# lacibeb/GA3C

Hardware: NVIDIA B200
Metric: TPS: A3C training frames/s, NetworkVP 84x84x4 (PPS: predictions/s, in 'pps') (higher is better)
Workload: dtype bf16

## Files before the change

### ga3c_b200/csrc/common.cuh

```cuda
#pragma once
#include <cuda_runtime.h>
#include <cuda_bf16.h>
#include <stdint.h>

namespace ga3c {

constexpr int IMG = 84, IMG_C = 4, STATE_DIM = IMG * IMG * IMG_C;
constexpr int C1_OUT = 16, H1 = 21, N1_POS = H1 * H1;
constexpr int C2_OUT = 32, H2 = 11, N2_POS = H2 * H2;
constexpr int FLAT = N2_POS * C2_OUT;
constexpr int FC = 256;
constexpr int MAX_ACTIONS = 18;

constexpr int XS_W = 88, XS_ROW_BYTES = XS_W * 8, XS_BYTES = XS_W * XS_ROW_BYTES;
constexpr int N1P_W = 24, N1P_BYTES = N1P_W * N1P_W * 32;

constexpr int XB_QROWS = 128, XB_QUARTERS = 4, XB_PLANE_BYTES = XB_QROWS * 16, XB_QBYTES = 8 * XB_PLANE_BYTES,
              XB_FRAME_BYTES = XB_QUARTERS * XB_QBYTES, XB_LIVE_ROWS = 484;
constexpr int G_W = 13, G_ROWS = 172, G_LBO = G_ROWS * 16, G_BYTES = 4 * G_LBO;
constexpr int B2_ROWS = 160, B2_LBO = B2_ROWS * 16, B2_BYTES = 8 * B2_LBO;
__host__ __device__ constexpr int b2_pixel_offset(int y, int x, int h) {
  return ((((y + 1) & 1) * 2 + ((x + 1) & 1)) * 2 + h) * B2_LBO + (((y + 1) >> 1) * G_W + ((x + 1) >> 1)) * 16;
}
__host__ __device__ constexpr int g_pos_offset(int oy, int ox, int j) { return j * G_LBO + ((oy + 1) * G_W + ox + 1) * 16; }

__device__ __forceinline__ uint32_t smem_u32(const void* p) {
  return static_cast<uint32_t>(__cvta_generic_to_shared(p));
}

__device__ __forceinline__ uint32_t pack_bf16(float lo, float hi) {
  __nv_bfloat162 v = __floats2bfloat162_rn(lo, hi);
  return *reinterpret_cast<uint32_t*>(&v);
}
__device__ __forceinline__ float bf16_lo(uint32_t v) { return __uint_as_float(v << 16); }
__device__ __forceinline__ float bf16_hi(uint32_t v) { return __uint_as_float(v & 0xFFFF0000u); }

__device__ __forceinline__ void mma_bf16_16816(float (&d)[4], const uint32_t (&a)[4], uint32_t b0, uint32_t b1) {
  asm volatile(
      "mma.sync.aligned.m16n8k16.row.col.f32.bf16.bf16.f32 {%0,%1,%2,%3}, {%4,%5,%6,%7}, {%8,%9}, {%0,%1,%2,%3};\n"
      : "+f"(d[0]), "+f"(d[1]), "+f"(d[2]), "+f"(d[3])
      : "r"(a[0]), "r"(a[1]), "r"(a[2]), "r"(a[3]), "r"(b0), "r"(b1));
}

__device__ __forceinline__ void ldsm_x4(uint32_t (&r)[4], uint32_t addr) {
  asm volatile("ldmatrix.sync.aligned.m8n8.x4.shared.b16 {%0,%1,%2,%3}, [%4];\n"
               : "=r"(r[0]), "=r"(r[1]), "=r"(r[2]), "=r"(r[3]) : "r"(addr));
}
__device__ __forceinline__ void ldsm_x4_t(uint32_t (&r)[4], uint32_t addr) {
  asm volatile("ldmatrix.sync.aligned.m8n8.x4.trans.shared.b16 {%0,%1,%2,%3}, [%4];\n"
               : "=r"(r[0]), "=r"(r[1]), "=r"(r[2]), "=r"(r[3]) : "r"(addr));
}
__device__ __forceinline__ void lds64(uint32_t& a, uint32_t& b, uint32_t addr) {
  asm volatile("ld.shared.v2.u32 {%0,%1}, [%2];\n" : "=r"(a), "=r"(b) : "r"(addr));
}
__device__ __forceinline__ void lds128(uint32_t (&r)[4], uint32_t addr) {
  asm volatile("ld.shared.v4.u32 {%0,%1,%2,%3}, [%4];\n"
               : "=r"(r[0]), "=r"(r[1]), "=r"(r[2]), "=r"(r[3]) : "r"(addr));
}
__device__ __forceinline__ void sts32(uint32_t addr, uint32_t v) {
  asm volatile("st.shared.u32 [%0], %1;\n" ::"r"(addr), "r"(v));
}
__device__ __forceinline__ void sts64(uint32_t addr, uint32_t a, uint32_t b) {
  asm volatile("st.shared.v2.u32 [%0], {%1,%2};\n" ::"r"(addr), "r"(a), "r"(b));
}
__device__ __forceinline__ void sts128(uint32_t addr, uint4 v) {
  asm volatile("st.shared.v4.u32 [%0], {%1,%2,%3,%4};\n" ::"r"(addr), "r"(v.x), "r"(v.y), "r"(v.z), "r"(v.w));
}

__device__ __forceinline__ void cp_async16(uint32_t dst, const void* src, int src_bytes) {
  asm volatile("cp.async.cg.shared.global [%0], [%1], 16, %2;\n" ::"r"(dst), "l"(src), "r"(src_bytes));
}
__device__ __forceinline__ void cp_async4(uint32_t dst, const void* src, int src_bytes) {
  asm volatile("cp.async.ca.shared.global [%0], [%1], 4, %2;\n" ::"r"(dst), "l"(src), "r"(src_bytes));
}
__device__ __forceinline__ void cp_async_commit() { asm volatile("cp.async.commit_group;\n" ::); }
template <int N>
__device__ __forceinline__ void cp_async_wait() { asm volatile("cp.async.wait_group %0;\n" ::"n"(N)); }

__device__ __forceinline__ float4 ldg_stream(const float4* p) {
  float4 r;
  asm volatile("ld.global.nc.L1::no_allocate.v4.f32 {%0,%1,%2,%3}, [%4];\n"
               : "=f"(r.x), "=f"(r.y), "=f"(r.z), "=f"(r.w) : "l"(p));
  return r;
}

__device__ __forceinline__ void mbar_init(uint32_t bar, uint32_t count) {
  asm volatile("mbarrier.init.shared::cta.b64 [%0], %1;\n" ::"r"(bar), "r"(count));
}
__device__ __forceinline__ void mbar_expect_tx(uint32_t bar, uint32_t bytes) {
  asm volatile("mbarrier.arrive.expect_tx.shared::cta.b64 _, [%0], %1;\n" ::"r"(bar), "r"(bytes) : "memory");
}
__device__ __forceinline__ void mbar_wait(uint32_t bar, uint32_t parity) {
  asm volatile(
      "{\n"
      ".reg .pred p;\n"
      "WAIT_%=:\n"
      "mbarrier.try_wait.parity.shared::cta.b64 p, [%0], %1;\n"
      "@p bra DONE_%=;\n"
      "bra WAIT_%=;\n"
      "DONE_%=:\n"
      "}\n" ::"r"(bar), "r"(parity) : "memory");
}
__device__ __forceinline__ void bulk_load(uint32_t dst, const void* src, uint32_t bytes, uint32_t bar) {
  asm volatile("cp.async.bulk.shared::cluster.global.mbarrier::complete_tx::bytes [%0], [%1], %2, [%3];\n" ::"r"(dst),
               "l"(src), "r"(bytes), "r"(bar)
               : "memory");
}
__device__ __forceinline__ uint64_t l2_policy_evict_first() {
  uint64_t p;
  asm volatile("createpolicy.fractional.L2::evict_first.b64 %0, 1.0;\n" : "=l"(p));
  return p;
}
__device__ __forceinline__ uint64_t l2_policy_evict_last() {
  uint64_t p;
  asm volatile("createpolicy.fractional.L2::evict_last.b64 %0, 1.0;\n" : "=l"(p));
  return p;
}
__device__ __forceinline__ uint64_t l2_policy_normal() {
  uint64_t p;
  asm volatile("createpolicy.fractional.L2::evict_normal.b64 %0, 1.0;\n" : "=l"(p));
  return p;
}
__device__ __forceinline__ void bulk_load_hint(uint32_t dst, const void* src, uint32_t bytes, uint32_t bar, uint64_t policy) {
  asm volatile("cp.async.bulk.shared::cluster.global.mbarrier::complete_tx::bytes.L2::cache_hint [%0], [%1], %2, [%3], %4;\n" ::"r"(dst),
               "l"(src), "r"(bytes), "r"(bar), "l"(policy)
               : "memory");
}
__device__ __forceinline__ void bulk_store_hint(void* dst, uint32_t src, uint32_t bytes, uint64_t policy) {
  asm volatile("cp.async.bulk.global.shared::cta.bulk_group.L2::cache_hint [%0], [%1], %2, %3;\n" ::"l"(dst), "r"(src), "r"(bytes),
               "l"(policy)
               : "memory");
}
__device__ __forceinline__ void stg128_hint(void* dst, uint4 v, uint64_t policy) {
  asm volatile("st.global.L2::cache_hint.v4.b32 [%0], {%1,%2,%3,%4}, %5;\n" ::"l"(dst), "r"(v.x), "r"(v.y), "r"(v.z), "r"(v.w), "l"(policy)
               : "memory");
}
__device__ __forceinline__ void bulk_store(void* dst, uint32_t src, uint32_t bytes) {
  asm volatile("cp.async.bulk.global.shared::cta.bulk_group [%0], [%1], %2;\n" ::"l"(dst), "r"(src), "r"(bytes) : "memory");
}
__device__ __forceinline__ void bulk_commit() { asm volatile("cp.async.bulk.commit_group;\n" ::: "memory"); }
__device__ __forceinline__ void bulk_wait_read0() { asm volatile("cp.async.bulk.wait_group.read 0;\n" ::: "memory"); }
__device__ __forceinline__ void fence_proxy_async() { asm volatile("fence.proxy.async.shared::cta;\n" ::: "memory"); }
__device__ __forceinline__ void fence_mbar_init() { asm volatile("fence.mbarrier_init.release.cluster;\n" ::: "memory"); }

constexpr int FRAME_BYTES = STATE_DIM * 4;
template <int NCH>
__device__ __forceinline__ void stg_issue_chunk(uint32_t stg, const float* frame, int c, uint32_t bars) {
  constexpr int CB = FRAME_BYTES / NCH, PARTS = 4 / NCH > 0 ? 4 / NCH : 1, PB = CB / PARTS;
  static_assert(CB * NCH == FRAME_BYTES && PB * PARTS == CB && PB % 16 == 0, "chunking must be exact and 16-B granular");
  mbar_expect_tx(bars + 8 * c, CB);
#pragma unroll
  for (int k = 0; k < PARTS; ++k)
    bulk_load(stg + c * CB + k * PB, reinterpret_cast<const uint8_t*>(frame) + c * CB + k * PB, PB, bars + 8 * c);
}

__device__ __forceinline__ void griddep_launch() { asm volatile("griddepcontrol.launch_dependents;\n" ::: "memory"); }

enum KernelId { K_CONV_FWD = 0, K_DENSE_FWD, K_HEADS, K_DENSE_WGRAD, K_DENSE_DGRAD, K_CONV12_BWD, K_CONV11_WGRAD, K_RMSPROP,
                K_GRAD_REDUCE, K_MLP_FUSED, K_MLP_WGRAD, K_MLP_REDUCE, K_DP_BIG, K_MLP_TC, K_HISTO,
                K_COUNT };
constexpr int TRACE_SLOTS = 6;
static __device__ unsigned long long* g_trace = nullptr;
__device__ __forceinline__ void trace_mark(int kid, int what) {
  if (threadIdx.x == 0) {
    unsigned long long* t = g_trace;
    if (t != nullptr) {
      unsigned long long now;
      asm volatile("mov.u64 %0, %%globaltimer;\n" : "=l"(now));
      atomicMin(t + kid * TRACE_SLOTS + 2 * what, now);
      atomicMax(t + kid * TRACE_SLOTS + 2 * what + 1, now);
    }
  }
}
__device__ __forceinline__ void trace_mark_by(int kid, int what, bool me) {
  if (me) {
    unsigned long long* t = g_trace;
    if (t != nullptr) {
      unsigned long long now;
      asm volatile("mov.u64 %0, %%globaltimer;\n" : "=l"(now));
      atomicMin(t + kid * TRACE_SLOTS + 2 * what, now);
      atomicMax(t + kid * TRACE_SLOTS + 2 * what + 1, now);
    }
  }
}
__device__ __forceinline__ void griddep_wait(int kid) {
  trace_mark(kid, 0);
  asm volatile("griddepcontrol.wait;\n" ::: "memory");
  trace_mark(kid, 1);
}
static __device__ unsigned long long* g_evt = nullptr;
constexpr unsigned int EVT_PER_WARP = 1024, EVT_WARPS = 16;
struct EvtLog {
  unsigned long long* base;
  unsigned int i;
};
__device__ __forceinline__ EvtLog evt_open() {
  EvtLog l;
  l.base = (blockIdx.x == 0 && (threadIdx.x & 31) == 0) ? g_evt : nullptr;
  l.i = 0;
  return l;
}
__device__ __forceinline__ void evt_mark(EvtLog& l, int id, int arg) {
  if (l.base != nullptr && l.i < EVT_PER_WARP) {
    unsigned long long now;
    asm volatile("mov.u64 %0, %%globaltimer;\n" : "=l"(now));
    const unsigned int slot = (threadIdx.x >> 5) * EVT_PER_WARP + l.i++;
    l.base[2 * slot] = now;
    l.base[2 * slot + 1] = ((unsigned long long)(threadIdx.x >> 5) << 32) | ((unsigned long long)id << 16) | (unsigned long long)(arg & 0xFFFF);
  }
}
#define GA3C_EVT_ATTACH(fn) \
  int fn(unsigned long long* buf) { return (int)cudaMemcpyToSymbol(g_evt, &buf, sizeof(buf)); }
#define GA3C_TRACE_ATTACH(fn)                                                                   \
  int fn(unsigned long long* buf) { return (int)cudaMemcpyToSymbol(g_trace, &buf, sizeof(buf)); }

template <class... KArgs, class... Args>
inline int launch_pdl(void (*kernel)(KArgs...), dim3 grid, dim3 block, size_t smem, cudaStream_t stream, Args... args) {
  cudaLaunchConfig_t cfg{};
  cfg.gridDim = grid; cfg.blockDim = block; cfg.dynamicSmemBytes = smem; cfg.stream = stream;
  cudaLaunchAttribute attr[1];
  attr[0].id = cudaLaunchAttributeProgrammaticStreamSerialization;
  attr[0].val.programmaticStreamSerializationAllowed = 1;
  cfg.attrs = attr; cfg.numAttrs = 1;
  return (int)cudaLaunchKernelEx(&cfg, kernel, static_cast<KArgs>(args)...);
}

__device__ __forceinline__ float warp_sum(float v) {
#pragma unroll
  for (int o = 16; o > 0; o >>= 1) v += __shfl_xor_sync(0xffffffffu, v, o);
  return v;
}

__device__ __forceinline__ int n1p_slot(int px) { return (px & ~7) | ((px >> 1) & 3) | ((px & 1) << 2); }
__device__ __forceinline__ int n1p_off(int py, int px, int chunk) {
  return ((py * N1P_W + n1p_slot(px)) << 5) + (((chunk ^ (px >> 3)) & 1) << 4);
}

template <int NT>
__device__ __forceinline__ void stage_frame_bf16(const float* __restrict__ x, uint32_t xs_base, int tid) {
  const float4* src = reinterpret_cast<const float4*>(x);
  constexpr int NPIX = IMG * IMG;
  constexpr int UNROLL = 7;
  for (int base = 0; base < NPIX; base += NT * UNROLL) {
    float4 v[UNROLL];
#pragma unroll
    for (int u = 0; u < UNROLL; ++u) {
      int i = base + u * NT + tid;
      if (i < NPIX) v[u] = ldg_stream(src + i);
    }
#pragma unroll
    for (int u = 0; u < UNROLL; ++u) {
      int i = base + u * NT + tid;
      if (i < NPIX) {
        int y = i / IMG, xx = i - y * IMG;
        sts64(xs_base + (y + 2) * XS_ROW_BYTES + (xx + 2) * 8, pack_bf16(v[u].x, v[u].y), pack_bf16(v[u].z, v[u].w));
      }
    }
  }
}

}
```

### ga3c_b200/csrc/conv_fwd.cu

```cuda
#include "common.cuh"
#include "kernels.h"
#include "tcgen05.cuh"
#include "conv_blk.cuh"

namespace ga3c {

constexpr int CF_THREADS = 512, CF_AUX_WARPS = 6, CF_ISSUE_WARP = 6, CF_STORE_WARP = 7, CF_EPI_WARP0 = 8;
static_assert(CF_EPI_WARP0 % 4 == 0, "epilogue warp e must own TMEM lane quarter e");
constexpr int C11_TILES = 4;
constexpr int C11_TSTRIDE = 127;
static_assert((C11_TILES - 1) * C11_TSTRIDE + 128 + BLK_W <= BLK_ROWS && C11_TILES * C11_TSTRIDE >= H1 * BLK_W, "tiles must cover the outputs and stay inside the buffer");

constexpr int CF_OFF_A2 = 0;
constexpr int CF_OFF_B2 = CF_OFF_A2 + 4 * 128 * 128;
constexpr int CF_OFF_BLK = CF_OFF_B2 + 4 * 32 * 128;
constexpr int CF_OFF_RING = CF_OFF_BLK + BLK_BYTES;
constexpr int CF_OFF_WQ = CF_OFF_RING + CF_AUX_WARPS * PW_SLOTS * PW_BYTES;
constexpr int CF_OFF_LUT = CF_OFF_WQ + 4 * 2048;
constexpr int CF_OFF_BIAS = CF_OFF_LUT + 3584;
constexpr int CF_OFF_BAR = CF_OFF_BIAS + (C1_OUT + C2_OUT) * 4;
constexpr int BAR_RING = 0;
constexpr int BAR_BLKRDY = 12;
constexpr int BAR_C11 = 16;
constexpr int BAR_T1FREE = 20;
constexpr int BAR_A2RDY = 24;
constexpr int BAR_MMA2 = 25;
constexpr int BAR_T2FREE = 26;
constexpr int BAR_STORED = 27;
constexpr int CF_NBAR = 31;
constexpr int CF_OFF_TSLOT = CF_OFF_BAR + CF_NBAR * 8;
constexpr int CF_OFF_XCH = CF_OFF_TSLOT + 16;
constexpr int CF_SMEM = CF_OFF_XCH + 1024 + 1024;
static_assert(CF_SMEM <= 232448, "shared memory budget of one CTA per SM");
constexpr int CF_TMEM_COLS = 256, TMEM_C12 = 128;

template <bool U8, bool EVT>
__global__ void __launch_bounds__(CF_THREADS, 1)
conv_fwd_kernel(const void* __restrict__ x, const float* __restrict__ w11, const float* __restrict__ b11,
                const float* __restrict__ w12, const float* __restrict__ b12,
                uint8_t* __restrict__ n1_out, uint8_t* __restrict__ xblk_out, uint16_t* __restrict__ n2_out, int batch, int hints) {
  extern __shared__ uint8_t smem_raw[];
  const uint32_t sbase = (smem_u32(smem_raw) + 1023u) & ~1023u;
  uint8_t* const smem = smem_raw + (sbase - smem_u32(smem_raw));
  const uint32_t sa2 = sbase + CF_OFF_A2, sb2 = sbase + CF_OFF_B2, blk = sbase + CF_OFF_BLK, ring = sbase + CF_OFF_RING,
                 wq = sbase + CF_OFF_WQ, lut = sbase + CF_OFF_LUT, bars = sbase + CF_OFF_BAR, tslot = sbase + CF_OFF_TSLOT;
  float* bias_s = reinterpret_cast<float*>(smem + CF_OFF_BIAS);
  const int tid = threadIdx.x, warp = tid >> 5, lane = tid & 31;
  EvtLog evt_i = EVT ? evt_open() : EvtLog{nullptr, 0};
  auto mark = [&](int id, int arg) { if (EVT) evt_mark(evt_i, id, arg); };
  const int stride = gridDim.x;
  const int n_frames = ((int)blockIdx.x < batch) ? (batch - 1 - (int)blockIdx.x) / stride + 1 : 0;
  const int n_chunks = n_frames * PW_NCHUNK;
  auto frame_of = [&](int k) { return (size_t)(blockIdx.x + k * stride); };
  auto bar = [&](int i) { return bars + i * 8; };
  const uint64_t pol_stream = (hints & 1) ? l2_policy_evict_first() : l2_policy_normal();
  const uint64_t pol_keep = (hints & 2) ? l2_policy_evict_last() : l2_policy_normal();
  auto issue_chunk = [&](int q, int slot) {
    const int k = q / PW_NCHUNK, c = q - k * PW_NCHUNK;
    constexpr uint32_t bytes = U8 ? PW_BYTES_U8 : PW_BYTES;
    mbar_expect_tx(bar(BAR_RING + slot), bytes);
    bulk_load_hint(ring + slot * PW_BYTES, static_cast<const uint8_t*>(x) + (frame_of(k) * PW_NCHUNK + c) * bytes, bytes,
                   bar(BAR_RING + slot), pol_stream);
  };

  mark(60, 0);
  if (tid == 0) {
    for (int i = 0; i < CF_AUX_WARPS * PW_SLOTS; ++i) mbar_init(bar(BAR_RING + i), 1);
    for (int i = 0; i < 4; ++i) {
      mbar_init(bar(BAR_BLKRDY + i), pw_group_chunks(i));
      mbar_init(bar(BAR_C11 + i), 1);
      mbar_init(bar(BAR_T1FREE + i), 4);
    }
    mbar_init(bar(BAR_A2RDY), 8);
    mbar_init(bar(BAR_MMA2), 1);
    mbar_init(bar(BAR_T2FREE), 4);
    for (int i = 0; i < 4; ++i) mbar_init(bar(BAR_STORED + i), 1);
    fence_mbar_init();
  }
  if (warp == CF_EPI_WARP0) tmem_alloc<CF_TMEM_COLS>(tslot);
  __syncthreads();
  mark(61, 0);
  if (warp < CF_AUX_WARPS && lane == 0)
    for (int j = 0; j < PW_SLOTS; ++j)
      if (warp + j * CF_AUX_WARPS < n_chunks) issue_chunk(warp + j * CF_AUX_WARPS, warp * PW_SLOTS + j);
  for (int i = tid; i < (CF_OFF_RING - CF_OFF_A2) / 16; i += CF_THREADS)
    if (i < CF_OFF_B2 / 16 || i >= CF_OFF_BLK / 16) sts128(sbase + i * 16, make_uint4(0, 0, 0, 0));
  for (int p = tid; p < N1_POS; p += CF_THREADS) {
    const int y = p / H1, xx = p - y * H1;
    uint32_t e[4];
#pragma unroll
    for (int idx = 0; idx < 4; ++idx) {
      const int kh = ((y + 1) & 1) + 2 * (idx >> 1), kw = ((xx + 1) & 1) + 2 * (idx & 1);
      const int oy2 = y + 1 - kh, ox2 = xx + 1 - kw;
      const bool ok = oy2 >= 0 && ox2 >= 0 && (oy2 >> 1) < H2 && (ox2 >> 1) < H2;
      const int row = kh * 128 + (oy2 >> 1) * H2 + (ox2 >> 1);
      e[idx] = ok ? (uint32_t)(row * 8 + ((2 * kw) ^ (row & 7))) : 0xFFFFu;
    }
    sts64(lut + p * 8, e[0] | (e[1] << 16), e[2] | (e[3] << 16));
  }
  fence_proxy_async();
  __syncthreads();
  mark(62, 0);
  griddep_launch();
  uint32_t tmem_base;
  asm volatile("ld.shared.u32 %0, [%1];\n" : "=r"(tmem_base) : "r"(tslot));
  if (warp >= CF_AUX_WARPS) {
    trace_mark_by(K_CONV_FWD, 0, tid == CF_AUX_WARPS * 32);
    asm volatile("griddepcontrol.wait;\n" ::: "memory");
    trace_mark_by(K_CONV_FWD, 1, tid == CF_AUX_WARPS * 32);
    mark(63, 0);
    const int t = tid - CF_AUX_WARPS * 32;
    float4 q12[8];
    float2 q11[8];
    const bool do12 = t < 256, do11 = t >= 64;
    const int kh = t >> 6, c12 = (t >> 3) & 7, n12 = (t & 7) * 4;
    if (do12) {
      const float* w = w12 + ((kh * 4 + (c12 >> 1)) * C1_OUT + (c12 & 1) * 8) * C2_OUT + n12;
#pragma unroll
      for (int e = 0; e < 8; ++e) q12[e] = *reinterpret_cast<const float4*>(w + e * C2_OUT);
    }
    const int i11 = t - 64, a11 = i11 >> 7, j11 = (i11 >> 4) & 7, b11i = (i11 >> 3) & 1, n11 = (i11 & 7) * 2;
    if (do11) {
      const float* w = w11 + (((4 * a11 + (j11 >> 1)) * 8 + 4 * b11i + (j11 & 1) * 2) * 4) * C1_OUT + n11;
#pragma unroll
      for (int e = 0; e < 8; ++e) q11[e] = *reinterpret_cast<const float2*>(w + e * C1_OUT);
    }
    if (t < C1_OUT) bias_s[t] = b11[t];
    if (t >= 32 && t < 32 + C2_OUT) bias_s[C1_OUT + t - 32] = b12[t - 32];
    if (do12) {
#pragma unroll
      for (int qn = 0; qn < 4; ++qn) {
        const int n = n12 + qn;
        auto f = [&](const float4& v) { return qn == 0 ? v.x : qn == 1 ? v.y : qn == 2 ? v.z : v.w; };
        sts128(sb2 + kh * 4096 + n * 128 + ((c12 ^ (n & 7)) << 4),
               make_uint4(pack_bf16(f(q12[0]), f(q12[1])), pack_bf16(f(q12[2]), f(q12[3])), pack_bf16(f(q12[4]), f(q12[5])),
                          pack_bf16(f(q12[6]), f(q12[7]))));
      }
    }
    if (do11) {
      const uint32_t dst = wq + a11 * 4096 + j11 * 512 + (b11i * 16 + n11) * 16;
      sts128(dst, make_uint4(pack_bf16(q11[0].x, q11[1].x), pack_bf16(q11[2].x, q11[3].x), pack_bf16(q11[4].x, q11[5].x),
                             pack_bf16(q11[6].x, q11[7].x)));
      sts128(dst + 16, make_uint4(pack_bf16(q11[0].y, q11[1].y), pack_bf16(q11[2].y, q11[3].y), pack_bf16(q11[4].y, q11[5].y),
                                  pack_bf16(q11[6].y, q11[7].y)));
    }
    fence_proxy_async();
    tc_fence_before();
    named_bar_sync(4, CF_THREADS - CF_AUX_WARPS * 32);
    tc_fence_after();
    mark(64, 0);
  }

  if (warp < CF_AUX_WARPS) {
    uint32_t lane_off[3];
    blk_lane_offsets(lane, lane_off);
    int j = 0;
#pragma unroll 1
    for (int q = warp; q < n_chunks; q += CF_AUX_WARPS, ++j) {
      const int k = q / PW_NCHUNK, c = q - k * PW_NCHUNK, slot = warp * PW_SLOTS + (j & 1);
      uint32_t pk[PW_ROWS][3][2];
      mbar_wait(bar(BAR_RING + slot), (j >> 1) & 1);
      blk_load_rows4<U8>(ring + slot * PW_BYTES, lane, pk);
      __syncwarp();
      if (lane == 0 && q + PW_SLOTS * CF_AUX_WARPS < n_chunks) issue_chunk(q + PW_SLOTS * CF_AUX_WARPS, slot);
      if (k > 0) {
        mbar_wait(bar(BAR_C11 + pw_last_consumer(c)), (k - 1) & 1);
        if (xblk_out != nullptr) mbar_wait(bar(BAR_STORED + pw_last_consumer(c)), (k - 1) & 1);
      }
      blk_store_rows4<BLK_LBO>(blk, c, lane, lane_off, pk);
      fence_proxy_async();
      __syncwarp();
      if (lane == 0) mbar_arrive(bar(BAR_BLKRDY + pw_first_consumer(c)));
    }
  } else if (warp == CF_ISSUE_WARP) {
    constexpr uint32_t idesc11 = make_idesc(2 * C1_OUT, false, false), idesc12 = make_idesc(C2_OUT, false, false);
    const uint32_t blk_k = desc_ns_lo(blk, BLK_LBO), wq_k = desc_ns_lo(wq, 512);
    constexpr uint32_t hi_k = desc_ns_hi(128);
    for (int k = 0; k < n_frames; ++k) {
#pragma unroll
      for (int i = 0; i < C11_TILES; ++i) {
        mbar_wait(bar(BAR_BLKRDY + i), k & 1);
        mark(15, k * 4 + i);
        if (k > 0) mbar_wait(bar(BAR_T1FREE + i), (k - 1) & 1);
        tc_fence_after();
        if (elect_one()) {
#pragma unroll
          for (int a = 0; a < 2; ++a)
#pragma unroll
            for (int kk = 0; kk < 4; ++kk)
              tc_mma_bf16_w(tmem_base + 32 * i, blk_k + C11_TSTRIDE * i + BLK_W * a + 2 * kk * (BLK_LBO / 16), hi_k,
                            wq_k + (a * 4096 + 2 * kk * 512) / 16, hi_k, idesc11, (a | kk) ? 1u : 0u);
          tc_commit(bar(BAR_C11 + i));
        }
        __syncwarp();
        mark(16, k * 4 + i);
      }
      mbar_wait(bar(BAR_A2RDY), k & 1);
      mark(17, k);
      if (k > 0) mbar_wait(bar(BAR_T2FREE), (k - 1) & 1);
      tc_fence_after();
      if (elect_one()) {
#pragma unroll
        for (int kb = 0; kb < 4; ++kb) {
          const uint64_t da = make_desc(sa2 + kb * 16384, false), db = make_desc(sb2 + kb * 4096, false);
#pragma unroll
          for (int kk = 0; kk < 4; ++kk)
            tc_mma_bf16(tmem_base + TMEM_C12, da + (uint64_t)(kk * 32 >> 4), db + (uint64_t)(kk * 32 >> 4), idesc12, (kb | kk) ? 1u : 0u);
        }
        tc_commit(bar(BAR_MMA2));
      }
      __syncwarp();
      mark(18, k);
    }
  } else if (warp == CF_STORE_WARP) {
    if (xblk_out != nullptr) {
      for (int k = 0; k < n_frames; ++k) {
        uint8_t* dst = xblk_out + frame_of(k) * XB_FRAME_BYTES;
#pragma unroll 1
        for (int q = 0; q < XB_QUARTERS; ++q) {
          mbar_wait(bar(BAR_BLKRDY + q), k & 1);
          if (lane < 8) {
            const uint32_t bytes = q < 3 ? XB_PLANE_BYTES : (XB_LIVE_ROWS - 3 * XB_QROWS) * 16;
            bulk_store_hint(dst + q * XB_QBYTES + lane * XB_PLANE_BYTES, blk + lane * BLK_LBO + q * XB_PLANE_BYTES, bytes, pol_keep);
            bulk_commit();
            bulk_wait_read0();
          }
          __syncwarp();
          if (lane == 0) mbar_arrive(bar(BAR_STORED + q));
        }
      }
      if (lane < 8) asm volatile("cp.async.bulk.wait_group 0;\n" ::: "memory");
    }
  } else if (warp >= CF_EPI_WARP0) {
    const int ew = warp & 3, eset = (warp - CF_EPI_WARP0) >> 2;
    const uint32_t tlane = tmem_base + ((uint32_t)(ew * 32) << 16);
    auto conv12_epilogue = [&](int k) {
      mbar_wait(bar(BAR_MMA2), k & 1);
      mark(43, k);
      tc_fence_after();
      uint32_t r[32];
      tc_ld32(tlane + TMEM_C12, r);
      tc_fence_before();
      __syncwarp();
      if (lane == 0) mbar_arrive(bar(BAR_T2FREE));
      const int pos = ew * 32 + lane;
      if (pos < N2_POS) {
        uint4* dst = reinterpret_cast<uint4*>(n2_out + frame_of(k) * FLAT + pos * C2_OUT);
#pragma unroll
        for (int i = 0; i < 4; ++i) {
          uint32_t o[4];
#pragma unroll
          for (int jj = 0; jj < 4; ++jj) {
            const int n = 8 * i + 2 * jj;
            o[jj] = pack_bf16(fmaxf(__uint_as_float(r[n]) + bias_s[C1_OUT + n], 0.f),
                              fmaxf(__uint_as_float(r[n + 1]) + bias_s[C1_OUT + n + 1], 0.f));
          }
          stg128_hint(dst + i, make_uint4(o[0], o[1], o[2], o[3]), pol_keep);
        }
      }
    };
    for (int k = 0; k < n_frames; ++k) {
      if (k > 0) {
        if (eset == 1) conv12_epilogue(k - 1);
        else mbar_wait(bar(BAR_MMA2), (k - 1) & 1);
      }
      mark(44, k);
      uint8_t* n1_dst = n1_out ? n1_out + frame_of(k) * B2_BYTES : nullptr;
#pragma unroll 1
      for (int i = eset; i < C11_TILES; i += 2) {
        mbar_wait(bar(BAR_C11 + i), k & 1);
        mark(40, k * 4 + i);
        tc_fence_after();
        uint32_t r[32];
        tc_ld32(tlane + 32 * i, r);
        tc_fence_before();
        __syncwarp();
        if (lane == 0) mbar_arrive(bar(BAR_T1FREE + i));
        float* xch = reinterpret_cast<float*>(smem + CF_OFF_XCH) + eset * 128 + ((i >> 1) & 1) * 64;
        if (lane == 0) {
#pragma unroll
          for (int c = 0; c < 16; ++c) xch[ew * 16 + c] = __uint_as_float(r[16 + c]);
        }
        named_bar_sync(2 + eset, 128);
        float up[16];
#pragma unroll
        for (int c = 0; c < 16; ++c) up[c] = __shfl_down_sync(0xffffffffu, __uint_as_float(r[16 + c]), 1);
        if (lane == 31 && ew < 3) {
#pragma unroll
          for (int c = 0; c < 16; ++c) up[c] = xch[(ew + 1) * 16 + c];
        }
        const int mt = ew * 32 + lane, m = C11_TSTRIDE * i + mt, oy = m / BLK_W, ox = m - oy * BLK_W;
        if (mt < C11_TSTRIDE && oy < H1 && ox < H1) {
          uint32_t o[8];
#pragma unroll
          for (int jj = 0; jj < 8; ++jj)
            o[jj] = pack_bf16(fmaxf(__uint_as_float(r[2 * jj]) + up[2 * jj] + bias_s[2 * jj], 0.f),
                              fmaxf(__uint_as_float(r[2 * jj + 1]) + up[2 * jj + 1] + bias_s[2 * jj + 1], 0.f));
          const uint4 lo = make_uint4(o[0], o[1], o[2], o[3]), hi = make_uint4(o[4], o[5], o[6], o[7]);
          const int p = oy * H1 + ox;
          uint32_t e01, e23;
          lds64(e01, e23, lut + p * 8);
          const uint32_t e[4] = {e01 & 0xFFFFu, e01 >> 16, e23 & 0xFFFFu, e23 >> 16};
#pragma unroll
          for (int idx = 0; idx < 4; ++idx) {
            if (e[idx] != 0xFFFFu) {
              sts128(sa2 + (e[idx] << 4), lo);
              sts128(sa2 + ((e[idx] ^ 1u) << 4), hi);
            }
          }
          if (n1_dst) {
            uint8_t* d = n1_dst + b2_pixel_offset(oy, ox, 0);
            stg128_hint(d, lo, pol_keep);
            stg128_hint(d + B2_LBO, hi, pol_keep);
          }
        }
      }
      fence_proxy_async();
      __syncwarp();
      if (lane == 0) mbar_arrive(bar(BAR_A2RDY));
      mark(42, k);
    }
    if (n_frames > 0 && eset == 1) conv12_epilogue(n_frames - 1);
  }

  tc_fence_before();
  __syncthreads();
  trace_mark(K_CONV_FWD, 2);
  if (warp == CF_EPI_WARP0) {
    tc_fence_after();
    tmem_dealloc<CF_TMEM_COLS>(tmem_base);
  }
}

GA3C_TRACE_ATTACH(trace_attach_conv_fwd)
static bool g_evt_attached_cf = false;
int evt_attach_conv_fwd(unsigned long long* buf) {
  g_evt_attached_cf = buf != nullptr;
  return (int)cudaMemcpyToSymbol(g_evt, &buf, sizeof(buf));
}

int configure_conv_fwd() {
  cudaError_t e = cudaFuncSetAttribute(conv_fwd_kernel<false, false>, cudaFuncAttributeMaxDynamicSharedMemorySize, CF_SMEM);
  if (e != cudaSuccess) return (int)e;
  e = cudaFuncSetAttribute(conv_fwd_kernel<true, false>, cudaFuncAttributeMaxDynamicSharedMemorySize, CF_SMEM);
  if (e != cudaSuccess) return (int)e;
  e = cudaFuncSetAttribute(conv_fwd_kernel<false, true>, cudaFuncAttributeMaxDynamicSharedMemorySize, CF_SMEM);
  if (e != cudaSuccess) return (int)e;
  return (int)cudaFuncSetAttribute(conv_fwd_kernel<true, true>, cudaFuncAttributeMaxDynamicSharedMemorySize, CF_SMEM);
}

int launch_conv_fwd(const void* x, bool x_u8, const float* w11, const float* b11, const float* w12, const float* b12,
                    uint8_t* n1_out, uint8_t* xblk_out, uint16_t* n2_out, int batch, int num_sms, cudaStream_t stream) {
  const int grid = min(batch, num_sms);
  const int hints = l2_hints(n1_out != nullptr, x_u8);
  auto kernel = x_u8 ? (g_evt_attached_cf ? conv_fwd_kernel<true, true> : conv_fwd_kernel<true, false>)
                     : (g_evt_attached_cf ? conv_fwd_kernel<false, true> : conv_fwd_kernel<false, false>);
  return launch_pdl(kernel, dim3(grid), dim3(CF_THREADS), CF_SMEM, stream, x, w11, b11, w12, b12, n1_out, xblk_out, n2_out, batch,
                    hints);
}

}
```

### ga3c_b200/csrc/net.cu

```cuda
#include <cstdio>
#include <cstdlib>
#include <cstring>
#include <mutex>
#include <string>
#include <vector>

#include "../../include/ga3c_b200.h"
#include "common.cuh"
#include "kernels.h"
#include "host_util.h"
#include "mlp.cuh"
#include "dp_exchange.cuh"

using namespace ga3c;

namespace {

thread_local std::string g_err;

int fail(const char* where, cudaError_t e) { return fail_cuda(where, e); }
int fail_msg(const std::string& m) { g_err = m; return -1; }

struct ParamDesc {
  std::string name;
// ... 680 lines not shown
  }
  LAUNCH(n, K_RMSPROP, (cudaStream_t)stream, launch_rmsprop_dual(d, (cudaStream_t)stream));
  n->global_step += 2;
  return 0;
}
extern "C" int ga3c_dual_forward_backward(ga3c_net* n, const float* x, const float* yr, const float* a, int32_t batch, float beta,
                                          float* loss, void* stream) {
  return dual_forward_backward_impl(n, x, false, yr, a, batch, beta, loss, stream);
}
extern "C" int ga3c_dual_forward_backward_u8(ga3c_net* n, const uint8_t* x, const float* yr, const float* a, int32_t batch,
                                             float beta, float* loss, void* stream) {
  return dual_forward_backward_impl(n, x, true, yr, a, batch, beta, loss, stream);
}
extern "C" int ga3c_dual_apply(ga3c_net* n, float lr, void* stream) { return dual_apply_impl(n, lr, stream); }

static DpBigArgs dp_big_args(ga3c_net* n, float lr, int n_exch) {
  DpBigArgs b{};
  for (int r = 0; r < n->dp_world; ++r) b.peer[r] = n->dp_peer[r];
  b.rank = n->dp_rank; b.world = n->dp_world; b.n_exch = n_exch; b.step = ++n->dp_step;
  b.arena_bytes = (int64_t)n->arena_floats * 4; b.shadow_off = 4 * b.arena_bytes; b.comm_offset = n->comm_off;
  b.w1_offset = n->off(P_D1W); b.w1_count = (int64_t)FLAT * FC;
  b.lr = lr; b.decay = n->cfg.rmsprop_decay; b.momentum = n->cfg.rmsprop_momentum; b.eps = n->cfg.rmsprop_epsilon;
  b.pushed = n->dp_exchange == 0 && n->dp_push;
  b.bigrecv_off = n->bigrecv_off;
  return b;
}
static RmsPropDpArgs dp_small_args(ga3c_net* n, float lr, int batch, const DpBigArgs& b) {
  RmsPropDpArgs d{};
  d.base = rmsprop_args(n, lr);
  d.base.preload = batch >= n->num_sms;
  for (int q = 0; q < n->dp_world; ++q) d.peer[q] = n->dp_peer[q];
  d.rank = n->dp_rank; d.world = n->dp_world; d.step = b.step;
  d.arena_bytes = b.arena_bytes; d.comm_offset = n->comm_off;
  d.has_red = 1; d.red = reduce_args(n, batch);
  return d;
}

static int train_step_empty(ga3c_net* n, float lr, float* loss, void* stream) {
  CK(cudaSetDevice(n->cfg.device));
  cudaStream_t st = (cudaStream_t)stream;
  if (n->cfg.dual_rmsprop || n->cfg.use_grad_clip)
    return fail_msg("ga3c_train_step: batch 0 is only defined for the peer-memory data-parallel step");
  n->gp_heads_grid = 0;
  n->loss_out = loss;
  n->last_batch = 0;
  if (n->dp_exchange == 4) {
    CK(cudaMemsetAsync(n->g + n->off(P_D1W), 0, (size_t)FLAT * FC * 4, st));
    DpBigArgs b = dp_big_args(n, lr, 0);
    b.pushed = 0;
    n->cur_exch = 0;
    CK(cudaEventRecord(n->dp_grad_ready, st));
    CK(cudaStreamWaitEvent(n->dp_stream, n->dp_grad_ready, 0));
    CKL(launch_dp_big_side(b, true, n->num_sms, n->dp_stream));
    n->log.launches++;
    CK(cudaEventRecord(n->dp_big_done, n->dp_stream));
    n->dp_big_pending = true;
    const RmsPropDpArgs d = dp_small_args(n, lr, 0, b);
    LAUNCH(n, K_RMSPROP, st, launch_dp_small(d, n->xbuf_off, st, false));
    n->global_step += 1;
    return 0;
  }
  if (n->dp_exchange == 0 || n->dp_exchange == 3) {
    CK(cudaMemsetAsync(n->g + n->off(P_D1W), 0, (size_t)FLAT * FC * 4, st));
    const DpBigArgs b = dp_big_args(n, lr, 0);
    n->cur_exch = 0;
    if (b.pushed) {
      CKL(launch_dp_push_zero(wgrad_push(n, b.step), (long long)FLAT * FC / 4, st));
      n->log.launches++;
    }
    const RmsPropDpArgs d = dp_small_args(n, lr, 0, b);
    LAUNCH(n, K_RMSPROP, st, launch_dp_tail(d, b, n->xbuf_off, n->num_sms, st));
    n->global_step += 1;
    return 0;
  }
  if (n->dp_exchange == 1) {
    CK(cudaMemsetAsync(n->g + n->off(P_D1W), 0, (size_t)FLAT * FC * 4, st));
    const DpBigArgs b = dp_big_args(n, lr, n->dp_exch);
    n->cur_exch = b.n_exch;
    float* gp = n->gpart;
    LAUNCH(n, K_CONV12_BWD, st, launch_conv_bwd(n->xblk, n->n1, n->dn2, n->w + n->off(P_C12W), nullptr,
                                                gp + n->off(P_C11W), gp + n->off(P_C11B), gp + n->off(P_C12W),
                                                gp + n->off(P_C12B), n->gp_stride, 0, n->num_sms, false, ConvBwdOpt{}, &b, st));
    const RmsPropDpArgs d = dp_small_args(n, lr, 0, b);
    n->cur_exch = 0;
    LAUNCH(n, K_RMSPROP, st, launch_dp_small(d, n->xbuf_off, st, true));
    n->global_step += 1;
    return 0;
  }
  CK(cudaMemsetAsync(n->g, 0, (size_t)n->arena_floats * 4, st));
  if (loss) CK(cudaMemsetAsync(loss, 0, 16, st));
  return apply_rmsprop_impl(n, lr, stream, nullptr);
}

static int train_step_impl(ga3c_net* n, const void* x, bool x_u8, const float* yr, const float* a, int32_t batch, float lr,
                           float beta, float* loss, void* stream) {
  if (n && batch == 0 && n->dp_world > 1) return train_step_empty(n, lr, loss, stream);
  if (n->cfg.dual_rmsprop) {
    if (n->dp_world > 1) return fail_msg("ga3c_train_step: DUAL_RMSPROP is not available with the peer-memory exchange (dp_mode 'nccl' is)");
    if (int r = dual_forward_backward_impl(n, x, x_u8, yr, a, batch, beta, loss, stream)) return r;
    return dual_apply_impl(n, lr, stream);
  }
  if (int r = fb_head_impl(n, x, x_u8, yr, a, batch, beta, loss, stream, false)) return r;
  if (n->cfg.use_grad_clip) {
    if (int r = fb_tail_impl(n, x, x_u8, batch, stream, true, true)) return r;
    return apply_rmsprop_impl(n, lr, stream, nullptr);
  }
  if (n->dp_world > 1 && n->dp_exchange == 4) {
    DpBigArgs b = dp_big_args(n, lr, 0);
    b.pushed = 0;
    n->cur_exch = 0;
    n->dp_side = &b;
    const int r = fb_tail_impl(n, x, x_u8, batch, stream, true, false);
    n->dp_side = nullptr;
    if (r) return r;
    RmsPropDpArgs d = dp_small_args(n, lr, batch, b);
    LAUNCH(n, K_RMSPROP, (cudaStream_t)stream, launch_dp_small(d, n->xbuf_off, (cudaStream_t)stream, false));
    n->global_step += 1;
    return 0;
  }
  if (n->dp_world > 1 && n->dp_exchange == 3) {
    const DpBigArgs b = dp_big_args(n, lr, 0);
    n->cur_exch = 0;
    ConvBwdOpt opt{};
    opt.mode = 2;
    if (int r = fb_tail_impl(n, x, x_u8, batch, stream, true, false, &b, nullptr, &opt)) return r;
    const RmsPropDpArgs d = dp_small_args(n, lr, batch, b);
    LAUNCH(n, K_RMSPROP, (cudaStream_t)stream, launch_dp_small(d, n->xbuf_off, (cudaStream_t)stream, true));
    n->global_step += 1;
    return 0;
  }
  if (n->dp_world > 1 && n->dp_exchange == 0) {
    const DpBigArgs b = dp_big_args(n, lr, 0);
    n->cur_exch = 0;
    if (int r = fb_tail_impl(n, x, x_u8, batch, stream, true, false, &b)) return r;
    const RmsPropDpArgs d = dp_small_args(n, lr, batch, b);
    LAUNCH(n, K_RMSPROP, (cudaStream_t)stream, launch_dp_tail(d, b, n->xbuf_off, n->num_sms, (cudaStream_t)stream));
    n->global_step += 1;
    return 0;
  }
  if (n->dp_world > 1 && n->dp_exchange == 1) {
    const DpBigArgs b = dp_big_args(n, lr, n->dp_exch);
    n->cur_exch = b.n_exch;
    int r = fb_tail_impl(n, x, x_u8, batch, stream, true, false, &b);
    const RmsPropDpArgs d = dp_small_args(n, lr, batch, b);
    n->cur_exch = 0;
    if (r) return r;
    LAUNCH(n, K_RMSPROP, (cudaStream_t)stream, launch_dp_small(d, n->xbuf_off, (cudaStream_t)stream, true));
    n->global_step += 1;
    return 0;
  }
  if (n->dp_world == 1 && n->fuse_opt) {
    ConvBwdOpt opt{};
    opt.mode = 1;
    opt.g = n->g + n->off(P_D1W); opt.w = n->w + n->off(P_D1W); opt.ms = n->ms + n->off(P_D1W); opt.mom = n->mom + n->off(P_D1W);
    opt.shadow = n->w1_shadow; opt.n4 = (long long)FLAT * FC / 4;
    opt.lr = lr; opt.decay = n->cfg.rmsprop_decay; opt.momentum = n->cfg.rmsprop_momentum; opt.eps = n->cfg.rmsprop_epsilon;
    if (int r = fb_tail_impl(n, x, x_u8, batch, stream, true, false, nullptr, nullptr, &opt)) return r;
    RmsPropArgs ra = rmsprop_args(n, lr);
    ra.n_floats = n->small_floats;
    ra.preload = batch >= n->num_sms;
    LAUNCH(n, K_RMSPROP, (cudaStream_t)stream, launch_rmsprop_reduce(ra, reduce_args(n, batch), (cudaStream_t)stream));
    n->global_step += 1;
    return 0;
  }
  if (int r = fb_tail_impl(n, x, x_u8, batch, stream, true, false)) return r;
  const GradReduceArgs red = reduce_args(n, batch);
  if (n->dp_world > 1)
    return apply_rmsprop_impl(n, lr, stream, &red);
  RmsPropArgs ra = rmsprop_args(n, lr);
  ra.preload = batch >= n->num_sms;
  LAUNCH(n, K_RMSPROP, (cudaStream_t)stream, launch_rmsprop_reduce(ra, red, (cudaStream_t)stream));
  n->global_step += 1;
  return 0;
}
extern "C" int ga3c_train_step(ga3c_net* n, const float* x, const float* yr, const float* a, int32_t batch, float lr,
                               float beta, float* loss, void* stream) {
  return train_step_impl(n, x, false, yr, a, batch, lr, beta, loss, stream);
}
extern "C" int ga3c_train_step_u8(ga3c_net* n, const uint8_t* x, const float* yr, const float* a, int32_t batch, float lr,
                                  float beta, float* loss, void* stream) {
  return train_step_impl(n, x, true, yr, a, batch, lr, beta, loss, stream);
}

extern "C" int ga3c_returns(const double* rewards, const int64_t* seg, int32_t n_segments, const double* terminal,
                            double discount, int32_t flags, double rmin, double rmax, double* out, void* stream) {
  if (n_segments < 0) return fail_msg("ga3c_returns: negative segment count");
  if (n_segments == 0) return 0;
  if (!rewards || !seg || !terminal || !out) return fail_msg("ga3c_returns: null buffer");
  CKL(launch_returns(rewards, seg, n_segments, terminal, discount, flags, rmin, rmax, out, (cudaStream_t)stream));
  return 0;
}

extern "C" int ga3c_select_actions(const float* p, const double* u, int32_t batch, int32_t na, int32_t* action,
                                   void* stream) {
  if (batch < 0) return fail_msg("ga3c_select_actions: negative batch");
  if (batch == 0) return 0;
  if (!p || !u || !action) return fail_msg("ga3c_select_actions: null buffer");
  if (na < 1 || na > MAX_ACTIONS) return fail_msg("ga3c_select_actions: num_actions must be 1..18");
  CKL(launch_select_actions(p, u, batch, na, action, (cudaStream_t)stream));
  return 0;
}

extern "C" int ga3c_workspace_ptr(ga3c_net* n, int which, void** ptr, int64_t* bytes) {
  if (!n || !ptr) return fail_msg("ga3c_workspace_ptr: null argument");
  const int64_t b = n->last_batch;
  switch (which) {
    case 0: *ptr = n->n1; if (bytes) *bytes = b * B2_BYTES; break;
    case 1: *ptr = n->n2; if (bytes) *bytes = b * FLAT * 2; break;
    case 2: *ptr = n->d1; if (bytes) *bytes = b * FC * 4; break;
    case 3: *ptr = n->dd1; if (bytes) *bytes = b * FC * 2; break;
    case 4: *ptr = n->dn2; if (bytes) *bytes = b * G_BYTES; break;
    case 5: *ptr = n->dn1; if (bytes) *bytes = b * N1_POS * C1_OUT * 2; break;
    case 6: *ptr = n->w1_shadow; if (bytes) *bytes = (int64_t)FLAT * FC * 2; break;
    case 7: *ptr = n->xblk; if (bytes) *bytes = b * XB_FRAME_BYTES; break;
    default: return fail_msg("ga3c_workspace_ptr: bad id");
  }
  return 0;
}

extern "C" int ga3c_histograms(ga3c_net* n, int32_t batch, const float* p, const float* v, double* out, int32_t* bad,
                               void* stream) {
  if (int r = check_batch(n, batch, "ga3c_histograms")) return r;
  if (!p || !v || !out || !bad) return fail_msg("ga3c_histograms: null buffer");
  if (batch != n->last_batch) return fail_msg("ga3c_histograms: batch differs from the last forward on this handle");
  if (n->dp_world > 1) return fail_msg("ga3c_histograms: not available on a peer-memory data-parallel handle");
  CK(cudaSetDevice(n->cfg.device));
  static_assert(GA3C_HISTO_SOURCES == P_COUNT + 5, "sources: the variables, n1, n2, d1, v, p");
  HistoArgs a{};
  for (int i = 0; i < P_COUNT; ++i) a.src[i] = HistoSrc{n->w + n->off(i), n->params[i].count, 0, 0};
  const long long b = batch;
  a.src[P_COUNT + 0] = HistoSrc{n->n1, b * B2_BYTES / 2, 1, 1};
  a.src[P_COUNT + 1] = HistoSrc{n->n2, b * FLAT, 1, 0};
  a.src[P_COUNT + 2] = HistoSrc{n->d1, b * FC, 0, 0};
  a.src[P_COUNT + 3] = HistoSrc{v, b, 0, 0};
  a.src[P_COUNT + 4] = HistoSrc{p, b * n->cfg.num_actions, 0, 0};
  a.n_src = GA3C_HISTO_SOURCES;
  a.out = out;
  a.bad = bad;
  if (int r = histo_plan(a)) return r;
  const size_t part_bytes = sizeof(double) * 4 * histo_blocks(a);
  if (part_bytes > n->histo_part_bytes) {
    CK(cudaFree(n->histo_part));
    n->histo_part = nullptr;
    n->histo_part_bytes = 0;
    CK(cudaMalloc((void**)&n->histo_part, part_bytes));
    n->histo_part_bytes = part_bytes;
  }
  a.part = n->histo_part;
  cudaStream_t st = (cudaStream_t)stream;
  if (int r = histo_zero(a, st)) return r;
  LAUNCH(n, K_HISTO, st, launch_histo(a, st));
  LAUNCH(n, K_HISTO, st, launch_histo_merge(a, st));
  return 0;
}

extern "C" int ga3c_keep_dn1(ga3c_net* n, int32_t on) {
  if (!n) return fail_msg("ga3c_keep_dn1: null handle");
  n->keep_dn1 = on != 0;
  return 0;
}

extern "C" int64_t ga3c_launch_count(const ga3c_net* n) { return n ? n->log.launches : 0; }

extern "C" int ga3c_kernel_count(void) { return K_COUNT; }
extern "C" const char* ga3c_kernel_name(int kid) { return (kid >= 0 && kid < K_COUNT) ? kKernelNames[kid] : nullptr; }

static int trace_attach_all(unsigned long long* buf) {
  int r;
  if ((r = trace_attach_conv_fwd(buf)) || (r = trace_attach_conv_bwd_fused(buf)) || (r = trace_attach_dense_tc(buf)) ||
      (r = trace_attach_heads(buf)) || (r = trace_attach_dense_heads(buf)) || (r = trace_attach_elementwise(buf)) || (r = trace_attach_mlp(buf)) || (r = trace_attach_mlp_tc(buf)) || (r = trace_attach_mlp_stream(buf)))
    return r;
  return 0;
}

extern "C" int ga3c_trace_begin(ga3c_net* n, void* stream) {
  if (!n) return fail_msg("ga3c_trace_begin: null handle");
  CK(cudaSetDevice(n->cfg.device));
  const size_t words = (size_t)K_COUNT * TRACE_SLOTS;
  if (!n->trace) CK(cudaMalloc((void**)&n->trace, words * 8));
  std::vector<unsigned long long> init(words);
  for (size_t i = 0; i < words; ++i) init[i] = (i & 1) ? 0ull : ~0ull;
  CK(cudaStreamSynchronize((cudaStream_t)stream));
  CK(cudaMemcpy(n->trace, init.data(), words * 8, cudaMemcpyHostToDevice));
  CKL(trace_attach_all(n->trace));
  return 0;
}

extern "C" int ga3c_trace_end(ga3c_net* n, uint64_t* stamps, int32_t n_kernels) {
  if (!n || !stamps || n_kernels < K_COUNT) return fail_msg("ga3c_trace_end: bad argument");
  if (!n->trace) return fail_msg("ga3c_trace_end: no trace in progress");
  CK(cudaSetDevice(n->cfg.device));
  CK(cudaDeviceSynchronize());
  CKL(trace_attach_all(nullptr));
  CK(cudaMemcpy(stamps, n->trace, (size_t)K_COUNT * TRACE_SLOTS * 8, cudaMemcpyDeviceToHost));
  return 0;
}

extern "C" int ga3c_evt_begin(ga3c_net* n) {
  if (!n) return fail_msg("ga3c_evt_begin: null handle");
  CK(cudaSetDevice(n->cfg.device));
  CK(cudaDeviceSynchronize());
  if (!n->evt) CK(cudaMalloc((void**)&n->evt, (size_t)2 * 16384 * 8));
  CK(cudaMemset(n->evt, 0, (size_t)2 * 16384 * 8));
  if (getenv("GA3C_EVT_DENSE") == nullptr) {
    CKL(evt_attach_conv_fwd(n->evt));
    CKL(evt_attach_conv_bwd(n->evt));
    CKL(evt_attach_elementwise(n->evt));
    CKL(evt_attach_dense_heads(n->evt));
  } else {
    CKL(evt_attach_dense_tc(n->evt));
  }
  return 0;
}

extern "C" int ga3c_evt_end(ga3c_net* n, uint64_t* records, int32_t cap, int32_t* count) {
  if (!n || !records || !count || !n->evt || cap < 16384) return fail_msg("ga3c_evt_end: bad argument");
  CK(cudaSetDevice(n->cfg.device));
  CK(cudaDeviceSynchronize());
  CKL(evt_attach_conv_fwd(nullptr));
  CKL(evt_attach_conv_bwd(nullptr));
  CKL(evt_attach_elementwise(nullptr));
  CKL(evt_attach_dense_heads(nullptr));
  CKL(evt_attach_dense_tc(nullptr));
  std::vector<uint64_t> all((size_t)2 * 16384);
  CK(cudaMemcpy(all.data(), n->evt, all.size() * 8, cudaMemcpyDeviceToHost));
  int32_t c = 0;
  for (int i = 0; i < 16384; ++i)
    if (all[2 * i] != 0) { records[2 * c] = all[2 * i]; records[2 * c + 1] = all[2 * i + 1]; ++c; }
  *count = c;
  return 0;
}

extern "C" int ga3c_timing_enable(ga3c_net* n, int32_t max_records) {
  if (!n || max_records < 0) return fail_msg("ga3c_timing_enable: bad argument");
  CK(cudaSetDevice(n->cfg.device));
  CK(cudaDeviceSynchronize());
  return n->log.enable(max_records);
}

extern "C" int ga3c_timing_collect(ga3c_net* n, double* total_ms, int64_t* counts, int32_t n_kernels) {
  if (!n || !total_ms || !counts || n_kernels < K_COUNT) return fail_msg("ga3c_timing_collect: bad argument");
  CK(cudaSetDevice(n->cfg.device));
  CK(cudaDeviceSynchronize());
  return n->log.collect(total_ms, reinterpret_cast<long long*>(counts), n_kernels);
}
```

Before: 10.44 million.

## Double-buffer conv1 TMEM accumulators and poll-schedule conv1/conv2 MMA issue

Doubles the TMEM allocation so conv1 tile accumulators alternate between two column banks by frame parity, with separate completion/free barriers per bank. The MMA issuing warp now polls barriers with test_wait and issues whichever of conv2 or the next conv1 tile is ready, instead of a fixed in-order sequence. This lets conv1 of the next frame proceed while the epilogue drains the previous frame, removing serialization stalls. It adds polling overhead with nanosleep and uses all 512 TMEM columns. It also adds extra event marks and an env option to trace only conv_fwd.

```diff
diff --git a/ga3c_b200/csrc/common.cuh b/ga3c_b200/csrc/common.cuh
--- a/ga3c_b200/csrc/common.cuh
+++ b/ga3c_b200/csrc/common.cuh
@@ -100,6 +100,16 @@
       "bra WAIT_%=;\n"
       "DONE_%=:\n"
       "}\n" ::"r"(bar), "r"(parity) : "memory");
+}
+__device__ __forceinline__ bool mbar_test(uint32_t bar, uint32_t parity) {
+  uint32_t done;
+  asm volatile(
+      "{\n"
+      ".reg .pred p;\n"
+      "mbarrier.test_wait.parity.shared::cta.b64 p, [%1], %2;\n"
+      "selp.u32 %0, 1, 0, p;\n"
+      "}\n" : "=r"(done) : "r"(bar), "r"(parity) : "memory");
+  return done != 0;
 }
 __device__ __forceinline__ void bulk_load(uint32_t dst, const void* src, uint32_t bytes, uint32_t bar) {
   asm volatile("cp.async.bulk.shared::cluster.global.mbarrier::complete_tx::bytes [%0], [%1], %2, [%3];\n" ::"r"(dst),
diff --git a/ga3c_b200/csrc/conv_fwd.cu b/ga3c_b200/csrc/conv_fwd.cu
--- a/ga3c_b200/csrc/conv_fwd.cu
+++ b/ga3c_b200/csrc/conv_fwd.cu
@@ -27,12 +27,14 @@
 constexpr int BAR_MMA2 = 25;
 constexpr int BAR_T2FREE = 26;
 constexpr int BAR_STORED = 27;
-constexpr int CF_NBAR = 31;
+constexpr int BAR_T1FREE_ODD = 31;
+constexpr int BAR_C11_ODD = 35;
+constexpr int CF_NBAR = 39;
 constexpr int CF_OFF_TSLOT = CF_OFF_BAR + CF_NBAR * 8;
 constexpr int CF_OFF_XCH = CF_OFF_TSLOT + 16;
 constexpr int CF_SMEM = CF_OFF_XCH + 1024 + 1024;
 static_assert(CF_SMEM <= 232448, "shared memory budget of one CTA per SM");
-constexpr int CF_TMEM_COLS = 256, TMEM_C12 = 128;
+constexpr int CF_TMEM_COLS = 512, TMEM_C12 = 128, TMEM_C11_ODD = 256;
 
 template <bool U8, bool EVT>
 __global__ void __launch_bounds__(CF_THREADS, 1)
@@ -53,11 +55,15 @@
   const int n_chunks = n_frames * PW_NCHUNK;
   auto frame_of = [&](int k) { return (size_t)(blockIdx.x + k * stride); };
   auto bar = [&](int i) { return bars + i * 8; };
+  auto c11_col = [](int k, int i) { return (uint32_t)((k & 1) * TMEM_C11_ODD + 32 * i); };
+  auto t1free = [&](int k, int i) { return bar(((k & 1) ? BAR_T1FREE_ODD : BAR_T1FREE) + i); };
+  auto c11done = [&](int k, int i) { return bar(((k & 1) ? BAR_C11_ODD : BAR_C11) + i); };
   const uint64_t pol_stream = (hints & 1) ? l2_policy_evict_first() : l2_policy_normal();
   const uint64_t pol_keep = (hints & 2) ? l2_policy_evict_last() : l2_policy_normal();
   auto issue_chunk = [&](int q, int slot) {
     const int k = q / PW_NCHUNK, c = q - k * PW_NCHUNK;
     constexpr uint32_t bytes = U8 ? PW_BYTES_U8 : PW_BYTES;
+    mark(70, q);
     mbar_expect_tx(bar(BAR_RING + slot), bytes);
     bulk_load_hint(ring + slot * PW_BYTES, static_cast<const uint8_t*>(x) + (frame_of(k) * PW_NCHUNK + c) * bytes, bytes,
                    bar(BAR_RING + slot), pol_stream);
@@ -69,7 +75,9 @@
     for (int i = 0; i < 4; ++i) {
       mbar_init(bar(BAR_BLKRDY + i), pw_group_chunks(i));
       mbar_init(bar(BAR_C11 + i), 1);
+      mbar_init(bar(BAR_C11_ODD + i), 1);
       mbar_init(bar(BAR_T1FREE + i), 4);
+      mbar_init(bar(BAR_T1FREE_ODD + i), 4);
     }
     mbar_init(bar(BAR_A2RDY), 8);
     mbar_init(bar(BAR_MMA2), 1);
@@ -159,14 +167,17 @@
     for (int q = warp; q < n_chunks; q += CF_AUX_WARPS, ++j) {
       const int k = q / PW_NCHUNK, c = q - k * PW_NCHUNK, slot = warp * PW_SLOTS + (j & 1);
       uint32_t pk[PW_ROWS][3][2];
+      mark(71, q);
       mbar_wait(bar(BAR_RING + slot), (j >> 1) & 1);
+      mark(72, q);
       blk_load_rows4<U8>(ring + slot * PW_BYTES, lane, pk);
       __syncwarp();
       if (lane == 0 && q + PW_SLOTS * CF_AUX_WARPS < n_chunks) issue_chunk(q + PW_SLOTS * CF_AUX_WARPS, slot);
       if (k > 0) {
-        mbar_wait(bar(BAR_C11 + pw_last_consumer(c)), (k - 1) & 1);
+        mbar_wait(c11done(k - 1, pw_last_consumer(c)), ((k - 1) >> 1) & 1);
         if (xblk_out != nullptr) mbar_wait(bar(BAR_STORED + pw_last_consumer(c)), (k - 1) & 1);
       }
+      mark(73, q);
       blk_store_rows4<BLK_LBO>(blk, c, lane, lane_off, pk);
       fence_proxy_async();
       __syncwarp();
@@ -176,41 +187,45 @@
     constexpr uint32_t idesc11 = make_idesc(2 * C1_OUT, false, false), idesc12 = make_idesc(C2_OUT, false, false);
     const uint32_t blk_k = desc_ns_lo(blk, BLK_LBO), wq_k = desc_ns_lo(wq, 512);
     constexpr uint32_t hi_k = desc_ns_hi(128);
-    for (int k = 0; k < n_frames; ++k) {
-#pragma unroll
-      for (int i = 0; i < C11_TILES; ++i) {
-        mbar_wait(bar(BAR_BLKRDY + i), k & 1);
-        mark(15, k * 4 + i);
-        if (k > 0) mbar_wait(bar(BAR_T1FREE + i), (k - 1) & 1);
+    auto ready = [&](bool local) { return __all_sync(0xffffffffu, local); };
+    int k11 = 0, i11 = 0;
+#pragma unroll 1
+    for (int k12 = 0; k12 < n_frames;) {
+      if (ready(mbar_test(bar(BAR_A2RDY), k12 & 1) && (k12 == 0 || mbar_test(bar(BAR_T2FREE), (k12 - 1) & 1)))) {
+        mark(17, k12);
         tc_fence_after();
         if (elect_one()) {
 #pragma unroll
+          for (int kb = 0; kb < 4; ++kb) {
+            const uint64_t da = make_desc(sa2 + kb * 16384, false), db = make_desc(sb2 + kb * 4096, false);
+#pragma unroll
+            for (int kk = 0; kk < 4; ++kk)
+              tc_mma_bf16(tmem_base + TMEM_C12, da + (uint64_t)(kk * 32 >> 4), db + (uint64_t)(kk * 32 >> 4), idesc12, (kb | kk) ? 1u : 0u);
+          }
+          tc_commit(bar(BAR_MMA2));
+        }
+        __syncwarp();
+        mark(18, k12);
+        ++k12;
+      } else if (k11 < n_frames &&
+                 ready(mbar_test(bar(BAR_BLKRDY + i11), k11 & 1) && (k11 < 2 || mbar_test(t1free(k11, i11), ((k11 >> 1) - 1) & 1)))) {
+        mark(15, k11 * 4 + i11);
+        tc_fence_after();
+        if (elect_one()) {
+#pragma unroll
           for (int a = 0; a < 2; ++a)
 #pragma unroll
             for (int kk = 0; kk < 4; ++kk)
-              tc_mma_bf16_w(tmem_base + 32 * i, blk_k + C11_TSTRIDE * i + BLK_W * a + 2 * kk * (BLK_LBO / 16), hi_k,
+              tc_mma_bf16_w(tmem_base + c11_col(k11, i11), blk_k + C11_TSTRIDE * i11 + BLK_W * a + 2 * kk * (BLK_LBO / 16), hi_k,
                             wq_k + (a * 4096 + 2 * kk * 512) / 16, hi_k, idesc11, (a | kk) ? 1u : 0u);
-          tc_commit(bar(BAR_C11 + i));
+          tc_commit(c11done(k11, i11));
         }
         __syncwarp();
-        mark(16, k * 4 + i);
-      }
-      mbar_wait(bar(BAR_A2RDY), k & 1);
-      mark(17, k);
-      if (k > 0) mbar_wait(bar(BAR_T2FREE), (k - 1) & 1);
-      tc_fence_after();
-      if (elect_one()) {
-#pragma unroll
-        for (int kb = 0; kb < 4; ++kb) {
-          const uint64_t da = make_desc(sa2 + kb * 16384, false), db = make_desc(sb2 + kb * 4096, false);
-#pragma unroll
-          for (int kk = 0; kk < 4; ++kk)
-            tc_mma_bf16(tmem_base + TMEM_C12, da + (uint64_t)(kk * 32 >> 4), db + (uint64_t)(kk * 32 >> 4), idesc12, (kb | kk) ? 1u : 0u);
-        }
-        tc_commit(bar(BAR_MMA2));
-      }
-      __syncwarp();
-      mark(18, k);
+        mark(16, k11 * 4 + i11);
+        if (++i11 == C11_TILES) { i11 = 0; ++k11; }
+      } else {
+        __nanosleep(32);
+      }
     }
   } else if (warp == CF_STORE_WARP) {
     if (xblk_out != nullptr) {
@@ -268,14 +283,14 @@
       uint8_t* n1_dst = n1_out ? n1_out + frame_of(k) * B2_BYTES : nullptr;
 #pragma unroll 1
       for (int i = eset; i < C11_TILES; i += 2) {
-        mbar_wait(bar(BAR_C11 + i), k & 1);
+        mbar_wait(c11done(k, i), (k >> 1) & 1);
         mark(40, k * 4 + i);
         tc_fence_after();
         uint32_t r[32];
-        tc_ld32(tlane + 32 * i, r);
+        tc_ld32(tlane + c11_col(k, i), r);
         tc_fence_before();
         __syncwarp();
-        if (lane == 0) mbar_arrive(bar(BAR_T1FREE + i));
+        if (lane == 0) mbar_arrive(t1free(k, i));
         float* xch = reinterpret_cast<float*>(smem + CF_OFF_XCH) + eset * 128 + ((i >> 1) & 1) * 64;
         if (lane == 0) {
 #pragma unroll
diff --git a/ga3c_b200/csrc/net.cu b/ga3c_b200/csrc/net.cu
--- a/ga3c_b200/csrc/net.cu
+++ b/ga3c_b200/csrc/net.cu
@@ -1006,7 +1006,9 @@
   CK(cudaDeviceSynchronize());
   if (!n->evt) CK(cudaMalloc((void**)&n->evt, (size_t)2 * 16384 * 8));
   CK(cudaMemset(n->evt, 0, (size_t)2 * 16384 * 8));
-  if (getenv("GA3C_EVT_DENSE") == nullptr) {
+  if (getenv("GA3C_EVT_CONV_FWD") != nullptr) {
+    CKL(evt_attach_conv_fwd(n->evt));
+  } else if (getenv("GA3C_EVT_DENSE") == nullptr) {
     CKL(evt_attach_conv_fwd(n->evt));
     CKL(evt_attach_conv_bwd(n->evt));
     CKL(evt_attach_elementwise(n->evt));
```

New measurement: 10.44 million (median of 6 runs). About the same (-0.0%).
